# AbbVie-ComputationalGenomics/SAIGEgds

Measured on AMD Instinct MI355X. Metric: variants/sec seqAssocGLMM_SPA at N=430K; achieved HBM GB/s vs roofline, higher is better.
Workload: dtype f64

## Files before the change

### saigegds_amd/csrc/host_lanes.h

```cpp
extern "C" int sgx_set_option(sgx_handle *h, const char *name, long long value)
{
	if (!h || !name) return fail(SGX_EINVAL, "sgx_set_option: NULL argument");
	const std::string n(name);
	if (n == "score_v1") h->force_v1 = value != 0;
	else if (n == "force_dense") h->force_dense = value != 0;
	else if (n == "spa_exact") h->force_exact = value != 0;
	else if (n == "pipe_mb") { if (value < 0 || value > 65536) return fail(SGX_EINVAL, "pipe_mb out of range"); h->pipe_bytes = (size_t)value << 20; return SGX_OK; }
	else if (n == "spa_scan_rows") h->spa_scan_rows = value != 0;
	else if (n == "guard_exp") { if (value < 0 || value > 300) return fail(SGX_EINVAL, "guard_exp must be 0..300"); h->guard_tol = std::pow(10.0, -(double)value); }
	else if (n == "three_plane") { if (value < -1 || value > 1) return fail(SGX_EINVAL, "three_plane must be -1 (automatic), 0 or 1"); h->dense_opt = (int)value; return SGX_OK; }
	else if (n == "lanes") {
		if (value < 1 || value > 4) return fail(SGX_EINVAL, "lanes must be 1..4");
		if (h->owner) return fail(SGX_EINVAL, "lanes: not on a twin");
		int rc = sgx_sync(h);
		if (rc) return rc;
		for (int i = (int)value - 1; i < 3; i++) if (h->twins[i]) { sgx_free(h->twins[i]); h->twins[i] = nullptr; }
		for (int i = 0; i < (int)value - 1; i++) {
			if (h->twins[i]) continue;
			std::unique_ptr<sgx_handle, void (*)(sgx_handle *)> t(new sgx_handle(), sgx_free);
			t->device = h->device; t->md = h->md; t->mf_ok = h->mf_ok; t->mfe = h->mfe; t->dQ = h->dQ;
			for (int g = 0; g < MF_MAXG; g++) { t->mf[g] = h->mf[g]; t->mf_nbfv[g] = h->mf_nbfv[g]; }
			t->owner = h;
			t->force_dense = h->force_dense; t->force_v1 = h->force_v1; t->force_exact = h->force_exact;
			t->spa_scan_rows = h->spa_scan_rows; t->guard_tol = h->guard_tol;
			rc = set_dev(t.get());
			if (!rc) rc = alloc_workspace(t.get());
			if (rc) return rc;
			h->twins[i] = t.release();
		}
		h->n_lanes = (int)value; h->next_lane = 0; h->last_issued = nullptr;
		return SGX_OK;
	}
	else return fail(SGX_EINVAL, "sgx_set_option: unknown option '%s'", name);
	for (sgx_handle *t : h->twins) if (t) { int rc = sgx_set_option(t, name, value); if (rc) return rc; }
	return SGX_OK;
}

static void stats_add(sgx_stats &into, const sgx_stats &x)
{
	into.n_variants += x.n_variants; into.n_valid += x.n_valid; into.n_spa += x.n_spa;
	into.n_spa_dense += x.n_spa_dense; into.n_spa_slow += x.n_spa_slow;
	into.ms_score += x.ms_score; into.ms_spa += x.ms_spa; into.ms_total += x.ms_total;
	into.ms_kernel += x.ms_kernel; into.ms_lists += x.ms_lists;
	into.score_launches += x.score_launches; into.spa_launches += x.spa_launches;
	into.three_plane += x.three_plane; into.n_unlisted += x.n_unlisted; into.n_guarded += x.n_guarded;
}

static int sync_lane(sgx_handle *h)
{
	int rc = set_dev(h);
	if (rc) return rc;
	HIPCHK(hipStreamSynchronize(h->stream));
	if (h->pend_dense.active) {
		h->pend_dense.active = false;
		if (h->stats_pending && h->h_counters[2] > 0) {
			rc = launch_pending_dense(h);
			if (rc) return rc;
			HIPCHK(hipStreamSynchronize(h->stream));
		}
	}
	if (h->stats_pending) {
		h->stats.n_spa = (uint64_t)(h->h_counters[0] + h->h_counters[7] - h->h_counters[6] + h->h_counters[5]);
		h->stats.n_valid = (uint64_t)h->h_counters[1];
		h->stats.n_spa_dense = (uint64_t)h->h_counters[2];
		h->stats.n_spa_slow = (uint64_t)h->h_counters[4];
		h->stats.three_plane = h->form == FORM_THREE ? 1u : 0u;
		h->stats.n_guarded = (uint32_t)h->h_counters[21];
		h->stats.n_unlisted = (uint32_t)h->h_counters[23] - h->stats.n_guarded;
		if (h->form != FORM_FP64) {
			sgx_handle *p = h->owner ? h->owner : h;
			const double frac = 64.0 * (double)h->h_counters[22] / ((double)std::max<uint64_t>(1, h->stats.n_variants) * (double)h->md.N);
			const bool over = (uint64_t)h->stats.n_unlisted * 32 > h->stats.n_variants;
			if (h->form != FORM_THREE && (frac > SGX_DENSE_ON || over)) p->dense_mode = true;
			else if (h->form == FORM_THREE && frac < SGX_DENSE_OFF) p->dense_mode = false;
		}
		float a = 0, b = 0, c = 0;
		(void)hipEventElapsedTime(&a, h->ev[0], h->ev[1]);
		(void)hipEventElapsedTime(&b, h->ev[1], h->ev[2]);
		(void)hipEventElapsedTime(&c, h->ev[0], h->ev[2]);
		h->stats.ms_score = a; h->stats.ms_spa = b; h->stats.ms_total = c;
		float k = 0;
		if (h->evk_set) (void)hipEventElapsedTime(&k, h->evk[0], h->evk[1]);
		h->stats.ms_kernel = k; h->evk_set = false;
		float l = 0;
		if (h->lists_timed) { (void)hipEventElapsedTime(&l, h->ev_lists, h->ev[0]); h->stats.ms_total += l; }
		h->stats.ms_lists = l; h->lists_timed = false;
		h->stats_pending = false;
		sgx_handle *p = h->owner ? h->owner : h;
		stats_add(p->total, h->stats);
		p->total_calls++;
	}
	return SGX_OK;
}

static int begin_call(sgx_handle *h)
{
	const int rc = sync_lane(h);
	if (rc) return rc;
	h->last_issued = h;
	return SGX_OK;
}

extern "C" int sgx_sync(sgx_handle *h)
{
	if (!h) return fail(SGX_EINVAL, "sgx_sync: NULL handle");
	int rc = sync_lane(h);
	for (sgx_handle *t : h->twins) if (!rc && t) rc = sync_lane(t);
	return rc;
}

extern "C" int sgx_get_stats(sgx_handle *h, sgx_stats *st)
{
	if (!h || !st) return fail(SGX_EINVAL, "sgx_get_stats: NULL argument");
	int rc = sgx_sync(h);
	if (rc) return rc;
	*st = (h->last_issued && h->last_issued != h) ? h->last_issued->stats : h->stats;
	return SGX_OK;
}

extern "C" int sgx_get_stats_total(sgx_handle *h, sgx_stats *st, uint64_t *n_calls, int reset)
{
	if (!h || !st) return fail(SGX_EINVAL, "sgx_get_stats_total: NULL argument");
	int rc = sgx_sync(h);
	if (rc) return rc;
	*st = h->total;
	if (n_calls) *n_calls = h->total_calls;
	if (reset) { h->total = sgx_stats{}; h->total_calls = 0; }
	return SGX_OK;
}
```

### saigegds_amd/csrc/host_spa.h

```cpp


template <int LO, typename F, int... I>
static bool with_int(int v, F &&f, std::integer_sequence<int, I...>)
{
	return ((v == LO + I && (f(std::integral_constant<int, LO + I>()), true)) || ...);
}
template <typename F>
static bool with_k(int K, F &&f) { return with_int<1>(K, f, std::make_integer_sequence<int, KMAX>()); }
template <typename F>
static void with_pp(int P, F &&f)
{
	if (P <= 8) f(std::integral_constant<int, 8>());
	else if (P <= 16) f(std::integral_constant<int, 16>());
	else if (P <= 32) f(std::integral_constant<int, 32>());
	else f(std::integral_constant<int, 64>());
}

static dim3 mf_grid(int n_cu, size_t rows, int ntile, int *tps, int vpb = MF_VPB, int wg_per_cu = 2)
{
	const int vt = (int)((rows + vpb - 1) / vpb);
	int sk = std::max(1, (n_cu * wg_per_cu * 4 + vt / 2) / vt);
	sk = std::min(sk, std::max(1, ntile / 24));
	if (sk >= 6) sk = (sk + 7) & ~7;
	sk = std::min(sk, std::max(1, ntile / 2));
	*tps = (ntile + sk - 1) / sk;
	*tps += *tps & 1;
	sk = (ntile + *tps - 1) / *tps;
	return dim3((unsigned)vt, (unsigned)sk);
}

template <int KK, int NCX, int INPUT>
static const void *spa4_moments_fn()
{
	if constexpr (INPUT == IN_2BIT) return (const void *)spa4_moments<KK, NCX>;
	else return (const void *)spa4_moments_ds<KK, NCX, INPUT>;
}

template <int KK, int INPUT>
static void launch_dense(sgx_handle *h, RowsRef rr, size_t M, int slot, const int *list, double *out8)
{
	const dim3 sgrid((unsigned)std::min<size_t>(M, (size_t)h->spa_grid));
	hipLaunchKernelGGL((spa_kernel<KK, 512, INPUT>), sgrid, dim3(512), 0, h->stream, rr,
		h->md, h->recs, h->counters, slot, list, h->scratch, h->scratch_stride, out8);
}

template <int KK, int INPUT>
static int launch_spa_k(sgx_handle *h, RowsRef rr, size_t M, double *out8, bool lazy_dense)
{
	const DevModel &md = h->md;
	hipStream_t st = h->stream;
	if (h->force_v1 && INPUT != IN_2BIT) {
		launch_dense<KK, INPUT>(h, rr, M, 0, nullptr, out8);
		return SGX_OK;
	}
	const size_t fl = spa4_lds_bytes(KK);
	if (!h->mom_attr_set[INPUT]) {
		HIPCHK(hipFuncSetAttribute(spa4_moments_fn<KK, SPA4_NCA, INPUT>(), hipFuncAttributeMaxDynamicSharedMemorySize, (int)fl));
		HIPCHK(hipFuncSetAttribute(spa4_moments_fn<KK, SPA4_NCB, INPUT>(), hipFuncAttributeMaxDynamicSharedMemorySize, (int)fl));
		h->mom_attr_set[INPUT] = true;
	}
	const int nround = (int)((M + h->vcap4 - 1) / h->vcap4);
	const int btop = (int)(2 * M);
	const dim3 gsolve((unsigned)std::min((h->vcap4 + 3) / 4, 4 * h->n_cu));
	const size_t rowb5 = (size_t)((md.N + 63) / 64) * 16;
	const size_t l5 = (INPUT == IN_2BIT && rowb5 <= 120 * 1024) ? rowb5 : 0;
	const bool small5 = INPUT == IN_2BIT && rowb5 <= 32 * 1024;
	if (l5 > 48 * 1024 && !h->spa5_attr_set[INPUT]) {
		HIPCHK(hipFuncSetAttribute((const void *)spa5_kernel<KK, INPUT, 0, 512>, hipFuncAttributeMaxDynamicSharedMemorySize, (int)l5));
		HIPCHK(hipFuncSetAttribute((const void *)spa5_kernel<KK, INPUT, 1, 512>, hipFuncAttributeMaxDynamicSharedMemorySize, (int)l5));
		h->spa5_attr_set[INPUT] = true;
	}
	auto moments = [&](auto ncx, int tier, int rd) {
		constexpr int NCX = decltype(ncx)::value;
		if constexpr (INPUT == IN_2BIT)
			hipLaunchKernelGGL((spa4_moments<KK, NCX>), dim3((unsigned)h->n_cu), dim3(WAVE * spa4_waves(KK)), fl, st, rr, md, h->nseg,
				tier, btop, rd * h->vcap4, h->vcap4, h->recs, h->counters, h->seg4, h->cur5 + 2);
		else
			hipLaunchKernelGGL((spa4_moments_ds<KK, NCX, INPUT>), dim3((unsigned)h->n_cu), dim3(WAVE * spa4_waves(KK)), fl, st,
				(const void *)rr.base, rr.bpv, md, h->nseg, tier, btop, rd * h->vcap4, h->vcap4, h->recs, h->counters, h->seg4, h->cur5 + 2);
		hipLaunchKernelGGL((spa4_solve<KK, NCX>), gsolve, dim3(256), 0, st, md, h->nseg, tier, btop, rd * h->vcap4, h->vcap4,
			h->recs, h->counters, h->seg4, h->fallback, h->fb_x2, out8, h->force_dense ? 1 : 0, h->force_exact ? 1 : 0);
	};
	for (int rd = 0; rd < nround; rd++) moments(std::integral_constant<int, SPA4_NCA>(), 0, rd);
	for (int rd = 0; rd < nround; rd++) moments(std::integral_constant<int, SPA4_NCB>(), 1, rd);
	const size_t ws5 = spa5_wg_bytes(md.N);
	auto spa5 = [&](auto threads, int nwg) {
		constexpr int T5 = decltype(threads)::value;
		if constexpr (T5 == 512 || INPUT == IN_2BIT) {
			hipLaunchKernelGGL((spa5_kernel<KK, INPUT, 0, T5>), dim3((unsigned)nwg), dim3(T5), l5, st, rr, md, h->recs, h->counters,
				h->fb_spa2, h->fb_x2, h->cur5, h->fallback, h->scr5, out8, h->force_dense ? 1 : 0, h->force_exact ? 1 : 0, l5,
				h->spa_scan_rows, ws5, 3);
			hipLaunchKernelGGL((spa5_kernel<KK, INPUT, 1, T5>), dim3((unsigned)nwg), dim3(T5), l5, st, rr, md, h->recs, h->counters,
				h->fb_x2, h->fb_x2, h->cur5 + 1, h->fallback, h->scr5, out8, h->force_dense ? 1 : 0, h->force_exact ? 1 : 0, l5,
				h->spa_scan_rows, ws5, 4);
		}
	};
	if (small5) spa5(std::integral_constant<int, 128>(), h->nwg5);
	else spa5(std::integral_constant<int, 512>(), h->n_cu);
	if (!lazy_dense) launch_dense<KK, INPUT>(h, rr, M, 2, h->fallback, out8);
	return SGX_OK;
}

template <int INPUT>
static int launch_spa(sgx_handle *h, RowsRef rr, size_t M, double *out8, bool lazy_dense = false)
{
	h->stats.spa_launches = 0;
	if (h->md.quant) return SGX_OK;
	int rc = SGX_OK;
	with_k(h->md.K, [&](auto kk) { rc = launch_spa_k<decltype(kk)::value, INPUT>(h, rr, M, out8, lazy_dense); });
	if (rc) return rc;
	HIPCHK(hipGetLastError());
	const bool v1 = h->force_v1 && INPUT != IN_2BIT;
	h->stats.spa_launches = v1 ? 1u : (uint32_t)(4 * ((M + h->vcap4 - 1) / h->vcap4) + 3);
	if (lazy_dense && !v1) { h->pend_dense.active = true; h->pend_dense.rr = rr; h->pend_dense.M = M; h->pend_dense.out8 = out8; }
	return SGX_OK;
}

static int launch_pending_dense(sgx_handle *h)
{
	with_k(h->md.K, [&](auto kk) {
		launch_dense<decltype(kk)::value, IN_2BIT>(h, h->pend_dense.rr, h->pend_dense.M, 2, h->fallback, h->pend_dense.out8);
	});
	HIPCHK(hipGetLastError());
	return SGX_OK;
}

static int scan_begin(sgx_handle *h, hipStream_t sst, ScanForm form, const sgx_block *b)
{
	h->form = form;
	if (b) HIPCHK(hipStreamWaitEvent(sst, b->ready, 0));
	if (form == FORM_FP64) {
		HIPCHK(hipMemsetAsync(h->counters, 0, 24 * sizeof(int), sst));
		if (h->cur5) HIPCHK(hipMemsetAsync(h->cur5, 0, 8 * sizeof(int), sst));
	}
	HIPCHK(hipEventRecord(h->ev[0], sst));
	return SGX_OK;
}

template <int INPUT>
static int scan_end(sgx_handle *h, hipStream_t sst, const sgx_block *b, RowsRef rr, size_t M, double *out8, bool lazy_dense)
{
	HIPCHK(hipEventRecord(h->ev[1], sst));
	h->stats.score_launches = h->form == FORM_FP64 ? 1 : 5;
	if (sst != h->stream) HIPCHK(hipStreamWaitEvent(h->stream, h->ev[1], 0));
	int rc = launch_spa<INPUT>(h, rr, M, out8, lazy_dense);
	if (rc) return rc;
	if (lazy_dense) h->pend_dense.blk = b;
	HIPCHK(hipEventRecord(h->ev[2], h->stream));
	if (b) {
		HIPCHK(hipEventRecord(b->last_read, h->stream));
		const_cast<sgx_block *>(b)->was_read = true;
	}
	HIPCHK(hipMemcpyAsync(h->h_counters, h->counters, 24 * sizeof(int), hipMemcpyDeviceToHost, h->stream));
	h->stats.n_variants = M;
	h->stats_pending = true;
	return SGX_OK;
}

template <int KK, int INPUT>
static int launch_score_fp64(sgx_handle *h, RowsRef rr, size_t M, double *out8, uint8_t *valid)
{
	const DevModel &md = h->md;
	constexpr int SB = 256, P = 2 * KK + 2;
	hipStream_t st = h->stream;
	const dim3 grid((unsigned)M);
	if constexpr (INPUT == IN_2BIT) {
		hipLaunchKernelGGL((score2b_kernel<P, SB>), grid, dim3(SB), 0, st,
			rr, (int)M, md, h->recs, h->counters, out8, valid, (const int *)nullptr, 0, 0, (int *)nullptr, (int *)nullptr);
	} else {
		using T = std::conditional_t<INPUT == IN_U8, uint8_t, double>;
		const T *rows = reinterpret_cast<const T *>(rr.base);
		if constexpr (KK <= 8) {
			if (!h->force_v1) {
				const int vb = (int)((M + DS_TILE_VB - 1) / DS_TILE_VB);
				int ns = std::max(1, std::min((4 * h->n_cu + vb - 1) / vb, (md.N + 4095) / 4096));
				int per = (((md.N + ns - 1) / ns) + 63) & ~63;
				ns = (md.N + per - 1) / per;
				const size_t need = (size_t)ns * M * (3 * P + 2);
				if (need > h->ds_part.cap) {
					HIPCHK(hipStreamSynchronize(st));
					HIPCHK(h->ds_part.reserve(need));
				}
				hipLaunchKernelGGL((score_ds_tile_kernel<P, T>), dim3((unsigned)vb, (unsigned)ns), dim3(256), 0, st,
					rows, (int)M, md, per, h->ds_part);
				hipLaunchKernelGGL((score_ds_tile_epilogue<P>), dim3((unsigned)((M + 255) / 256)), dim3(256), 0, st,
					(int)M, md, ns, h->ds_part, h->recs, h->counters, out8, valid);
				return SGX_OK;
			}
		}
		hipLaunchKernelGGL((score_ds_kernel<P, SB, T>), grid, dim3(SB), 0, st, rows, (int)M, md, h->recs, h->counters, out8, valid);
	}
	return SGX_OK;
}

template <int INPUT>
static int launch_scan(sgx_handle *h, const void *rows, size_t row_bytes, size_t M, double *out8, uint8_t *valid,
	const sgx_block *b = nullptr)
{
	const RowsRef rr{reinterpret_cast<const uint8_t *>(rows), row_bytes, 0, nullptr, nullptr, nullptr};
	int rc = scan_begin(h, h->stream, FORM_FP64, b);
	if (rc) return rc;
	if (!with_k(h->md.K, [&](auto kk) { rc = launch_score_fp64<decltype(kk)::value, INPUT>(h, rr, M, out8, valid); }))
		return fail(SGX_EINVAL, "unsupported K=%d", h->md.K);
	if (rc) return rc;
	HIPCHK(hipGetLastError());
	return scan_end<INPUT>(h, h->stream, b, rr, M, out8, false);
}
```

### saigegds_amd/csrc/kern_spa4.h

```cpp
#pragma once
#include "kern_spa4_tab.h"


__host__ __device__ constexpr int spa4_waves(int) { return 8; }
#define SPA4_NCA 12
#define SPA4_NCB SPA4_NC
#define SPA4_NSMAX (SPA4_NC + 5)
#define SPA4_TAIL_TOL 1e-10

__device__ __forceinline__ double spa4_fma_svv(double a_sgpr, double x, double c_vgpr)
{
	double r;
	asm("v_fma_f64 %0, %1, %2, %3" : "=v"(r) : "s"(a_sgpr), "v"(x), "v"(c_vgpr));
	return r;
}

__device__ __forceinline__ void spa4_max_abs(double &g, double a)
{
	asm("v_max_f64 %0, %0, |%1|" : "+v"(g) : "v"(a));
}

template <int NC>
__device__ __forceinline__ void spa4_cum_terms(double y, double u, double d, double *acc)
{
// ... 260 lines not shown
				};
				fetch_q(ca, lane);
				for (int k0 = 0; k0 < nq; k0 += 2 * WAVE) {
					fetch_q(cb, k0 + WAVE + lane);
					if (ca.ok) work(ca);
					fetch_q(ca, k0 + 2 * WAVE + lane);
					if (cb.ok) work(cb);
				}
				__builtin_amdgcn_wave_barrier();
				fetch(ca);
				while (__ballot(ca.ok)) {
					fetch(cb);
					if (ca.ok) work(ca);
					ca = cb;
				}
			}
			const int idx = wave_reduce_scatter(acc, lane);
			gmax = wave_max_nonneg_to_last(gmax);
			const size_t base = ((size_t)(vb + vl) * nseg + seg) * NS;
			if (!(lane & (NS - 1 > 16 ? 1 : 3)) && idx < NS - 1) segpart[base + idx] = acc[0];
			if (lane == WAVE - 1) segpart[base + (NS - 1)] = gmax;
		}
	}
	spa4_queue_done(cursor);
}

template <int K, int NC, int INPUT>
__global__ void __launch_bounds__(WAVE * spa4_waves(K))
spa4_moments_ds(const void *__restrict__ rows, size_t row_bytes, DevModel md, int nseg, int tier, int btop, int v0, int vcap,
	const SpaRec *__restrict__ recs, const int *__restrict__ counters, double *__restrict__ segpart, int *__restrict__ cursor)
{
	constexpr int SEG = spa_seg(K), KP = (K + 2) & ~1, NS = NC + 5;
	extern __shared__ __attribute__((aligned(16))) uint8_t fill_smem[];
	double *tab = reinterpret_cast<double *>(fill_smem);
	double *pd = tab + (size_t)SEG * KP;
	int *pj = reinterpret_cast<int *>(pd + (size_t)(K + 6) * SPA4_VPER);
	const int N = md.N, tid = threadIdx.x, lane = tid & (WAVE - 1), wid = tid / WAVE;
	const int nflag = min(counters[tier ? 7 : 0] - v0, vcap);
	if (nflag <= 0) return;
	const int vper = spa4_slice(nflag, nseg, gridDim.x, spa4_waves(K));
	const int nslice = (nflag + vper - 1) / vper;
	const int nitem = nseg * nslice;
	__shared__ int sh_it;
	int seg = -1;
	for (;;) {
		__syncthreads();
		if (tid == 0) sh_it = atomicAdd(cursor, 1);
		__syncthreads();
		const int it = sh_it;
		if (it >= nitem) break;
		const int sg = it / nslice, vb = (it - sg * nslice) * vper;
		const int nv = min(vper, nflag - vb);
		if (sg != seg) {
			seg = sg;
			const int nrow = min(SEG, N - seg * SEG);
			spa4_stage_table<spa4_waves(K)>(tab, md.XM + (size_t)seg * SEG * KP, nrow * KP);
		}
		for (int i = tid; i < nv; i += WAVE * spa4_waves(K)) {
			const SpaRec &r = recs[spa4_rec(tier, btop, v0 + vb + i)];
			pj[i] = r.j;
			pj[SPA4_VPER + i] = r.minus;
			pd[i] = 1 / sqrt(r.AC2);
			pd[SPA4_VPER + i] = r.tscale;
#pragma unroll
			for (int a = 0; a < K; a++) pd[(2 + a) * SPA4_VPER + i] = r.c[a];
#pragma unroll
			for (int a = 0; a < 4; a++) pd[(2 + K + a) * SPA4_VPER + i] = r.lut[a];
		}
		__syncthreads();
		const int s_lo = seg * SEG, nstep = (min(SEG, N - s_lo) + WAVE - 1) / WAVE;
		for (int vl = wid; vl < nv; vl += spa4_waves(K)) {
			const double inv = pd[vl], ts = pd[SPA4_VPER + vl];
			const double imp = pd[(2 + K + 3) * SPA4_VPER + vl];
			const bool minus = pj[SPA4_VPER + vl] != 0;
			const uint8_t *row = reinterpret_cast<const uint8_t *>(rows) + (size_t)pj[vl] * row_bytes;
			double c[K];
#pragma unroll
			for (int a = 0; a < K; a++) c[a] = pd[(2 + a) * SPA4_VPER + vl];
			double acc[NS - 1], gmax = 0;
#pragma unroll
			for (int a = 0; a < NS - 1; a++) acc[a] = 0;
			auto dosage = [&](int j) -> double {
				const int i = s_lo + j * WAVE + lane;
				if (i >= N) return 0.0;
				if (INPUT == IN_U8) {
					const uint8_t v = row[i];
					return (v == 0xFF) ? imp : (minus ? 2.0 - (double)v : (double)v);
				} else {
					const double v = reinterpret_cast<const double *>(row)[i];
					return !isfinite(v) ? imp : (minus ? 2.0 - v : v);
				}
			};
			double gn = dosage(0);
			for (int j = 0; j < nstep; j++) {
				const double G = gn;
				if (j + 1 < nstep) gn = dosage(j + 1);
				if (G != 0) spa4_carrier<K, NC>(tab + (size_t)(j * WAVE + lane) * KP, G, c, inv, ts, acc, gmax);
			}
			const int idx = wave_reduce_scatter(acc, lane);
			gmax = wave_max_nonneg_to_last(gmax);
			const size_t base = ((size_t)(vb + vl) * nseg + seg) * NS;
			if (!(lane & (NS - 1 > 16 ? 1 : 3)) && idx < NS - 1) segpart[base + idx] = acc[0];
			if (lane == WAVE - 1) segpart[base + (NS - 1)] = gmax;
		}
	}
	spa4_queue_done(cursor);
}

template <int NC>
struct Spa4Series {
	double k1, k2;
	double kp[NC - 2];
	double ts, gmax;
};

template <int NC>
__device__ __forceinline__ bool spa4_eval(const Spa4Series<NC> &S, double xmax, double t, double &K1s, double &K2s, double &K0s)
{
	const double its = 1 / S.ts, tau = t * its;
	double p0 = 0, p1 = 0, p2 = 0;
#pragma unroll
	for (int n = NC; n >= 3; n--) {
		const double kn = S.kp[n - 3];
		p0 = fma(p0, tau, kn);
		p1 = fma(p1, tau, (double)n * kn);
		p2 = fma(p2, tau, (double)(n * (n - 1)) * kn);
	}
	const double tau2 = tau * tau;
	K0s = fma(t, S.k1, fma(0.5 * t * t, S.k2, p0 * tau2 * tau));
	K1s = S.k1 + fma(t, S.k2, p1 * tau2 * its);
	K2s = fma(p2 * tau, its * its, S.k2);
	double tp = tau;
#pragma unroll
	for (int k = 1; k < NC - 3; k++) tp *= tau;
	const double tail = (fabs((double)(NC * (NC - 1)) * S.kp[NC - 3] * tp * tau) +
		fabs((double)((NC - 1) * (NC - 2)) * S.kp[NC - 4] * tp)) * its * its;
	return S.gmax * fabs(t) <= xmax && tail <= SPA4_TAIL_TOL * fabs(K2s) && isfinite(K2s);
}

template <int NC>
__device__ __forceinline__ bool spa4_root(const Spa4Series<NC> &S, double xmax, double q, double NAmu, double NAsigma, RootState &s)
{
	root_begin(s, q, 0, 0);
	root_feed(s, S.k1, S.k2, NAmu, NAsigma, 0.0, true);
	while (s.active) {
		double K1s, K2s, K0s;
		if (!spa4_eval(S, xmax, s.tnew, K1s, K2s, K0s)) return false;
		root_feed(s, K1s, K2s, NAmu, NAsigma, K0s, true);
	}
	return true;
}

template <int K, int NC>
__device__ __forceinline__ void spa4_solve_one(const DevModel &md, int nseg, int tier, int btop, int v0, int vcap, int v, int lane,
	SpaRec *__restrict__ recs, int *__restrict__ counters, const double *__restrict__ segpart,
	int *__restrict__ fb_dense, int *__restrict__ fb_exact, double *__restrict__ out8, int force_dense, int force_exact);

template <int K, int NC>
__global__ void __launch_bounds__(256)
spa4_solve(DevModel md, int nseg, int tier, int btop, int v0, int vcap, SpaRec *__restrict__ recs, int *__restrict__ counters,
	const double *__restrict__ segpart, int *__restrict__ fb_dense, int *__restrict__ fb_exact,
	double *__restrict__ out8, int force_dense, int force_exact)
{
	const int lane = threadIdx.x & (WAVE - 1);
	const int nflag = min(counters[tier ? 7 : 0] - v0, vcap);
	for (int v = (blockIdx.x * blockDim.x + threadIdx.x) / WAVE; v < nflag; v += gridDim.x * blockDim.x / WAVE)
		spa4_solve_one<K, NC>(md, nseg, tier, btop, v0, vcap, v, lane, recs, counters, segpart, fb_dense, fb_exact, out8,
			force_dense, force_exact);
}

template <int K, int NC>
__device__ __forceinline__ void spa4_solve_one(const DevModel &md, int nseg, int tier, int btop, int v0, int vcap, int v, int lane,
	SpaRec *__restrict__ recs, int *__restrict__ counters, const double *__restrict__ segpart,
	int *__restrict__ fb_dense, int *__restrict__ fb_exact, double *__restrict__ out8, int force_dense, int force_exact)
{
	constexpr int NS = NC + 5;
	const int ri = spa4_rec(tier, btop, v0 + v);
	const SpaRec r = recs[ri];
	double a[NS];
#pragma unroll
	for (int x = 0; x < NS; x++) a[x] = 0;
	for (int s = lane; s < nseg; s += WAVE) {
		const double *p = segpart + ((size_t)v * nseg + s) * NS;
#pragma unroll
		for (int x = 0; x < NS - 1; x++) a[x] += p[x];
		a[NS - 1] = fmax(a[NS - 1], p[NS - 1]);
	}
#pragma unroll
	for (int x = 0; x < NS - 1; x++) a[x] = wave_sum(a[x]);
#pragma unroll
	for (int o = 32; o > 0; o >>= 1) a[NS - 1] = fmax(a[NS - 1], __shfl_xor(a[NS - 1], o, WAVE));
	if (lane > 1) return;
	const double inv = 1 / sqrt(r.AC2);
	double xmu_c = 0, xsum_c = 0;
#pragma unroll
	for (int x = 0; x < K; x++) { xmu_c = fma(md.Xmu[x], r.c[x], xmu_c); xsum_c = fma(md.Xsum[x], r.c[x], xsum_c); }
	const double Tstat = r.S * inv;
	const double var2 = r.var2 / r.AC2, var1 = var2 * md.r;
	const double m1 = (a[0] - xmu_c) * inv;
	const double qtilde = Tstat / sqrt(var1) * sqrt(var2) + m1;
	const double sdev = qtilde - m1, qinv = -sdev + m1;
	const double pn_in = d_pchisq1_upper(sdev * sdev / var2);
	if (fabs(qtilde - m1) / sqrt(var2) < 2.0) {
		if (lane == 0) spa_write_row(r, Tstat, var1, pn_in, true, out8);
		return;
	}
	const double nb = (xsum_c - a[1]) * inv;
	const double L = a[2] + fmax(-nb, 0.0), U = a[3] + fmin(-nb, 0.0);
	const double mar = 1e-9 * (fabs(L) + fabs(U) + fabs(qtilde) + fabs(qinv));
	if (force_dense || !(qtilde < L - mar && qtilde > U + mar && qinv < L - mar && qinv > U + mar)) {
		if (lane == 0) fb_dense[atomicAdd(&counters[2], 1)] = ri;
		return;
	}
	Spa4Series<NC> S;
	S.k1 = a[4]; S.k2 = a[5]; S.ts = r.tscale; S.gmax = a[NS - 1];
#pragma unroll
	for (int x = 0; x < NC - 2; x++) S.kp[x] = a[6 + x];
	const double NAmu = m1 - a[4], NAsigma = var2 - a[5];
	const double qmine = lane == 0 ? qtilde : qinv;
	RootState sm;
	const bool ok_mine = !force_exact && spa4_root(S, md.spa_xmax, qmine, NAmu, NAsigma, sm);
	double p_mine = 0;
	if (ok_mine && sm.converged) p_mine = lugannani_rice(sm.root, sm.Kcur, sm.K2cur, qmine, NAmu, NAsigma);
	const int st_mine = (ok_mine ? 1 : 0) | (ok_mine && sm.converged ? 2 : 0);
	const double p_other = __shfl(p_mine, 1, WAVE);
	const int st_other = __shfl(st_mine, 1, WAVE);
	if (lane != 0) return;
	if (!(st_mine & 1) || !(st_other & 1)) {
		if (tier == 0 && !force_exact) {
			const int slot = atomicAdd(&counters[7], 1);
			atomicAdd(&counters[6], 1);
			recs[btop - 1 - slot] = r;
		} else {
			fb_exact[atomicAdd(&counters[4], 1)] = ri;
		}
		return;
	}
	bool converged;
	const double pval = spa_two_roots(p_mine, p_other, (st_mine & 2) && (st_other & 2), pn_in, converged);
	spa_write_row(r, Tstat, var1, pval, converged, out8);
}


#define SPA5_BIG 2048

__device__ __forceinline__ void cgf_terms_rt(double g, double m, double t, bool with_k, double &k1, double &k2, double &k0)
{
	const double om = 1 - m, mg = m * g, c2 = om * mg * g;
	const double e = fast_exp(-g * t);
	const double d = fma(om, e, m);
	const double rr = isfinite(d) ? fast_rcp(d) : 0.0;
	k1 = fma(mg, rr, k1);
	const double tt = c2 * e * rr * rr;
	if (isfinite(tt)) k2 += tt;
	if (with_k) k0 += cgf_korg_term(g, m, t, d, om);
}

__host__ __device__ inline size_t spa5_wg_bytes(int N) { return (((size_t)N + 63) & ~(size_t)63) * (16 + 4); }

template <int BLOCK>
__device__ __noinline__ void spa5_cum_sweep(const double2 *__restrict__ glist, int nnz, double ts, double *kp_out)
{
	constexpr int NC = SPA4_NCB;
	double kp[NC - 1];
#pragma unroll
	for (int a = 0; a < NC - 1; a++) kp[a] = 0;
	double2 gn = (int)threadIdx.x < nnz ? glist[threadIdx.x] : make_double2(0.0, 0.5);
	for (int k = threadIdx.x; k < nnz; k += BLOCK) {
		const double2 gm = gn;
		if (k + BLOCK < nnz) gn = glist[k + BLOCK];
		const double mui = gm.y;
		spa4_cum_terms<NC>(gm.x * ts, mui * (1 - mui), 1 - 2 * mui, kp);
		kp[NC - 2] = fmax(kp[NC - 2], fabs(gm.x));
	}
#pragma unroll
	for (int a = 0; a < NC - 1; a++) kp_out[a] = kp[a];
}

__device__ __noinline__ int spa5_series_solve(const double *arg, const SpaRec *__restrict__ rec, double *__restrict__ out8)
{
	constexpr int NC = SPA4_NCB;
	Spa4Series<NC> S;
#pragma unroll
	for (int a = 0; a < NC - 2; a++) S.kp[a] = arg[a];
	S.k1 = arg[NC - 2]; S.k2 = arg[NC - 1]; S.ts = arg[NC]; S.gmax = arg[NC + 1];
	const double xmax = arg[NC + 2], qtilde = arg[NC + 3], qinv = arg[NC + 4], NAmu = arg[NC + 5], NAsigma = arg[NC + 6];
	const double pn_in = arg[NC + 7], Tstat = arg[NC + 8], var1 = arg[NC + 9];
	RootState s1, s2;
	if (!spa4_root(S, xmax, qtilde, NAmu, NAsigma, s1) || !spa4_root(S, xmax, qinv, NAmu, NAsigma, s2)) return 0;
	const bool both = s1.converged && s2.converged;
	double p1 = 0, p2 = 0;
	if (both) {
		p1 = lugannani_rice(s1.root, s1.Kcur, s1.K2cur, qtilde, NAmu, NAsigma);
		p2 = lugannani_rice(s2.root, s2.Kcur, s2.K2cur, qinv, NAmu, NAsigma);
	}
	bool converged;
	const double pval = spa_two_roots(p1, p2, both, pn_in, converged);
	const SpaRec rr = *rec;
	spa_write_row(rr, Tstat, var1, pval, converged, out8);
	return 1;
}

template <int BLOCK>
__device__ __forceinline__ bool spa5_series(const double2 *__restrict__ glist, int nnz, double ts, double xmax,
	double k1, double k2, double qtilde, double qinv, double NAmu, double NAsigma, double pn_in,
	double Tstat, double var1, const SpaRec *__restrict__ rec, double *__restrict__ out8, double *sh, int *sh_flag)
{
	constexpr int NC = SPA4_NCB;
	double kp[NC - 1];
	spa5_cum_sweep<BLOCK>(glist, nnz, ts, kp);
	constexpr int NWV = BLOCK / WAVE;
	double gmax = kp[NC - 2];
	const int lane = threadIdx.x & (WAVE - 1), wv = threadIdx.x / WAVE;
	double kr[NC - 2];
#pragma unroll
	for (int a = 0; a < NC - 2; a++) kr[a] = kp[a];
	const int idx = wave_reduce_scatter(kr, lane);
#pragma unroll
	for (int o = 32; o > 0; o >>= 1) gmax = fmax(gmax, __shfl_xor(gmax, o, WAVE));
	double *part = sh + NC + 16;
	if (!(lane & 3) && idx < NC - 2) part[idx * NWV + wv] = kr[0];
	if (lane == 1) part[(NC - 2) * NWV + wv] = gmax;
	__syncthreads();
	double *arg = sh;
	if (threadIdx.x < NC - 2) {
		double t = 0;
		for (int w = 0; w < NWV; w++) t += part[threadIdx.x * NWV + w];
		arg[threadIdx.x] = t;
	}
	__syncthreads();
	if (threadIdx.x == 0) {
		for (int w = 0; w < NWV; w++) gmax = fmax(gmax, part[(NC - 2) * NWV + w]);
		arg[NC - 2] = k1; arg[NC - 1] = k2; arg[NC] = ts; arg[NC + 1] = gmax; arg[NC + 2] = xmax;
		arg[NC + 3] = qtilde; arg[NC + 4] = qinv; arg[NC + 5] = NAmu; arg[NC + 6] = NAsigma;
		arg[NC + 7] = pn_in; arg[NC + 8] = Tstat; arg[NC + 9] = var1;
		*sh_flag = spa5_series_solve(arg, rec, out8);
	}
	__syncthreads();
	const bool done = *sh_flag != 0;
	__syncthreads();
	return done;
}

__host__ __device__ constexpr int spa5_waves_per_simd(int BLOCK) { return BLOCK == 512 ? 2 : (BLOCK / 64 + 3) / 4; }
template <int K, int INPUT, int MODE, int BLOCK>
__global__ void __launch_bounds__(BLOCK, spa5_waves_per_simd(BLOCK))
spa5_kernel(RowsRef rr, DevModel md, const SpaRec *__restrict__ recs,
	int *__restrict__ counters, const int *__restrict__ todo, int *__restrict__ todo_next, int *__restrict__ cursor,
	int *__restrict__ fb_dense, uint8_t *__restrict__ scratch, double *__restrict__ out8, int force_dense, int force_exact,
	size_t lds_row_bytes, bool scan_rows, size_t wg_stride, int nslot)
{
	constexpr int KP = (K + 2) & ~1, NW = BLOCK / WAVE;
	extern __shared__ __attribute__((aligned(16))) uint8_t fill_smem[];
	uint4 *rows_lds = reinterpret_cast<uint4 *>(fill_smem);
	__shared__ double sh[SPA4_NCB * NW + SPA4_NCB + 16];
	__shared__ int sh_flag;
	__shared__ int shi[NW];
	__shared__ int sh_vi, sh_v;
	__shared__ SpaRec sh_rec;
	const int N = md.N, tid = threadIdx.x, lane = tid & (WAVE - 1), wid = tid / WAVE;
	double2 *glist = reinterpret_cast<double2 *>(scratch + (size_t)blockIdx.x * wg_stride);
	uint32_t *ilist = reinterpret_cast<uint32_t *>(glist + (((size_t)N + 63) & ~(size_t)63));
	const int ntodo = counters[nslot];
	const int nvec = INPUT == IN_2BIT ? (int)(min((size_t)((N + 63) >> 6) * 16, rr_row_bytes(rr)) / 16) : (N + 63) >> 6;
	const int per = ((nvec + NW - 1) / NW + WAVE - 1) & ~(WAVE - 1);
	for (;;) {
		__syncthreads();
		if (tid < WAVE) {
			int vi0 = 0;
			if (tid == 0) vi0 = atomicAdd(cursor, 1);
			vi0 = __builtin_amdgcn_readfirstlane(vi0);
			int v0 = -1;
			if (vi0 < 2 * ntodo) {
				v0 = todo[vi0 < ntodo ? vi0 : vi0 - ntodo];
				const double *src = reinterpret_cast<const double *>(recs + v0);
				for (int i = tid; i < (int)(sizeof(SpaRec) / 8); i += WAVE) reinterpret_cast<double *>(&sh_rec)[i] = src[i];
			}
			if (tid == 0) { sh_vi = vi0; sh_v = v0; }
		}
		__syncthreads();
		const int vi = sh_vi;
		if (vi >= 2 * ntodo) break;
		const bool big_round = vi < ntodo;
		const int v = sh_v;
		const SpaRec &r = sh_rec;
		if ((r.nnz > SPA5_BIG) != big_round) continue;
		auto row_piece = [&](int p) -> uint4 { return *reinterpret_cast<const uint4 *>(rr.base + rr_piece(rr, (size_t)r.j, (size_t)p)); };
		const uint32_t zx = r.minus ? 0xAAAAAAAAu : 0u;
		const double lut0 = r.lut[0], lut1 = r.lut[1], lut2 = r.lut[2], lut3 = r.lut[3];
		const bool listed = INPUT == IN_2BIT && !scan_rows && rr.cptr != nullptr && rr.corient[r.j] == (r.minus ? 2 : 1);
		const uint32_t *il = listed ? rr.cidx + rr.cptr[r.j] : ilist;
		int nnz = listed ? r.nnz : 0;
		if (!listed) {
			const bool staged = INPUT == IN_2BIT && lds_row_bytes >= (size_t)nvec * 16;
			if (staged) {
				constexpr int UN = 8;
				for (int p0 = tid; p0 < nvec; p0 += UN * BLOCK) {
					uint4 t[UN];
	#pragma unroll
					for (int j = 0; j < UN; j++) { const int p = p0 + j * BLOCK; t[j] = p < nvec ? row_piece(p) : make_uint4(0u, 0u, 0u, 0u); }
	#pragma unroll
					for (int j = 0; j < UN; j++) { const int p = p0 + j * BLOCK; if (p < nvec) rows_lds[p] = t[j]; }
				}
				__syncthreads();
			}
			auto masks = [&](int p, uint32_t (&ww)[4], uint32_t (&z)[4]) -> int {
				int cnt = 0;
				if (INPUT == IN_2BIT) {
					uint4 w = make_uint4(0u, 0u, 0u, 0u);
					if (p < nvec) w = staged ? rows_lds[p] : row_piece(p);
					ww[0] = w.x; ww[1] = w.y; ww[2] = w.z; ww[3] = w.w;
	#pragma unroll
					for (int k = 0; k < 4; k++) { z[k] = nz_fields((ww[k] ^ zx) & keep_mask(N - p * 64 - 16 * k)); cnt += __popc(z[k]); }
				} else {
					z[0] = z[1] = z[2] = z[3] = 0;
					if (p < nvec) {
						for (int s2 = 0; s2 < 64; s2++) {
							const int i = p * 64 + s2;
							if (i < N && load_dosage<INPUT>(rr, i, r) != 0) { z[s2 >> 5] |= 1u << (s2 & 31); cnt++; }
						}
					}
				}
				return cnt;
			};
			int cnt_w = 0;
			for (int it = 0; it < per; it += WAVE) {
				uint32_t ww[4], z[4];
				cnt_w += masks(wid * per + it + lane, ww, z);
			}
			cnt_w = wave_sum_i(cnt_w);
			if (lane == 0) shi[wid] = cnt_w;
			__syncthreads();
			int o_w = 0;
	#pragma unroll
			for (int w = 0; w < NW; w++) { if (w < wid) o_w += shi[w]; nnz += shi[w]; }
			for (int it = 0; it < per; it += WAVE) {
				uint32_t ww[4], z[4];
				const int p = wid * per + it + lane;
				const int cnt = masks(p, ww, z);
				if (!__ballot(cnt != 0)) continue;
				int incl = cnt;
	#pragma unroll
				for (int o = 1; o < WAVE; o <<= 1) {
					const int up = __shfl_up(incl, o, WAVE);
					if (lane >= o) incl += up;
				}
				int o2 = o_w + incl - cnt;
				o_w += __shfl(incl, WAVE - 1, WAVE);
				if (INPUT == IN_2BIT) {
	#pragma unroll
					for (int k = 0; k < 4; k++) {
						uint32_t zz = z[k];
						while (zz) {
							const int b = __ffs(zz) - 1;
							zz &= zz - 1;
							ilist[o2++] = (uint32_t)(p * 64 + 16 * k + (b >> 1)) | (((ww[k] >> b) & 3u) << 30);
						}
					}
				} else {
	#pragma unroll
					for (int k = 0; k < 2; k++) {
						uint32_t zz = z[k];
						while (zz) {
							const int b = __ffs(zz) - 1;
							zz &= zz - 1;
							ilist[o2++] = (uint32_t)(p * 64 + 32 * k + b);
						}
					}
				}
			}
			__syncthreads();
		}
		const double inv = 1 / sqrt(r.AC2);
		double c[K];
#pragma unroll
		for (int a = 0; a < K; a++) c[a] = r.c[a];
		double a6[6] = {0, 0, 0, 0, 0, 0};
		constexpr int UNG = K <= 4 ? 4 : 2;
		for (int k0 = tid; k0 < nnz; k0 += UNG * BLOCK) {
			uint32_t e[UNG];
			double xv[UNG][KP];
#pragma unroll
			for (int j = 0; j < UNG; j++) e[j] = (k0 + j * BLOCK < nnz) ? il[k0 + j * BLOCK] : 0u;
#pragma unroll
			for (int j = 0; j < UNG; j++) {
				const double *x = md.XM + (size_t)(e[j] & 0x3FFFFFFFu) * KP;
#pragma unroll
				for (int a = 0; a < KP; a += 2) {
					const double2 t2 = *reinterpret_cast<const double2 *>(x + a);
					xv[j][a] = t2.x; xv[j][a + 1] = t2.y;
				}
			}
#pragma unroll
			for (int j = 0; j < UNG; j++) {
				const int k = k0 + j * BLOCK;
				if (k >= nnz) continue;
				const uint32_t code = e[j] >> 30;
				const double G = INPUT == IN_2BIT ? ((code & 2u) ? ((code & 1u) ? lut3 : lut2) : ((code & 1u) ? lut1 : lut0))
					: load_dosage<INPUT>(rr, (int)(e[j] & 0x3FFFFFFFu), r);
				double b = 0;
#pragma unroll
				for (int a = 0; a < K; a++) b = fma(xv[j][a], c[a], b);
				const double mui = xv[j][K];
				const double adj = (G - b) * inv;
				glist[k] = make_double2(adj, mui);
				a6[0] = fma(mui, G, a6[0]);
				a6[1] += b;
				if (adj > 0) a6[2] += adj; else a6[3] += adj;
				a6[4] = fma(adj, mui, a6[4]);
				a6[5] = fma(adj * adj, mui * (1 - mui), a6[5]);
			}
		}
		block_sum<6, BLOCK>(a6, sh);
		double xmu_c = 0, xsum_c = 0;
#pragma unroll
		for (int a = 0; a < K; a++) { xmu_c = fma(md.Xmu[a], c[a], xmu_c); xsum_c = fma(md.Xsum[a], c[a], xsum_c); }
		const double m1 = (a6[0] - xmu_c) * inv;
		const double Tstat = r.S * inv;
		const double var2 = r.var2 / r.AC2, var1 = var2 * md.r;
		const double qtilde = Tstat / sqrt(var1) * sqrt(var2) + m1;
		const double sdev = qtilde - m1, qinv = -sdev + m1;
		const double pn_in = d_pchisq1_upper(sdev * sdev / var2);
		double pval;
		bool converged = true;
		if (fabs(qtilde - m1) / sqrt(var2) < 2.0) {
			pval = pn_in;
		} else {
			const double nb = (xsum_c - a6[1]) * inv;
			const double L = a6[2] + fmax(-nb, 0.0), U = a6[3] + fmin(-nb, 0.0);
			const double mar = 1e-9 * (fabs(L) + fabs(U) + fabs(qtilde) + fabs(qinv));
			if (force_dense || !(qtilde < L - mar && qtilde > U + mar && qinv < L - mar && qinv > U + mar)) {
				if (tid == 0) fb_dense[atomicAdd(&counters[2], 1)] = v;
				continue;
			}
			const double NAmu = m1 - a6[4], NAsigma = var2 - a6[5];
			if (MODE == 0) {
				if (force_exact || !spa5_series<BLOCK>(glist, nnz, r.tscale, md.spa_xmax, a6[4], a6[5], qtilde, qinv, NAmu, NAsigma,
						pn_in, Tstat, var1, &sh_rec, out8, sh, &sh_flag)) {
					if (tid == 0) todo_next[atomicAdd(&counters[4], 1)] = v;
				}
				continue;
			}
			RootState s1, s2;
			root_begin(s1, qtilde, L, U);
			root_begin(s2, qinv, L, U);
			root_feed(s1, a6[4], a6[5], NAmu, NAsigma, 0.0, true);
			root_feed(s2, a6[4], a6[5], NAmu, NAsigma, 0.0, true);
			auto sweep = [&](bool a1, bool a2, bool k1w, bool k2w, double t1, double t2, double (&sv)[6]) {
#pragma unroll
				for (int a = 0; a < 6; a++) sv[a] = 0;
				double2 gn = tid < nnz ? glist[tid] : make_double2(0.0, 0.5);
				for (int k0 = tid; k0 < nnz; k0 += BLOCK) {
					const double2 gm = gn;
					if (k0 + BLOCK < nnz) gn = glist[k0 + BLOCK];
					if (a1) cgf_terms_rt(gm.x, gm.y, t1, k1w, sv[0], sv[1], sv[2]);
					if (a2) cgf_terms_rt(gm.x, gm.y, t2, k2w, sv[3], sv[4], sv[5]);
				}
				block_sum<6, BLOCK>(sv, sh);
			};
			while (s1.active || s2.active) {
				const bool a1 = s1.active, a2 = s2.active, k1w = s1.want_k, k2w = s2.want_k;
				double sv[6];
				sweep(a1, a2, k1w, k2w, s1.tnew, s2.tnew, sv);
				if (a1) root_feed(s1, sv[0], sv[1], NAmu, NAsigma, sv[2], k1w);
				if (a2) root_feed(s2, sv[3], sv[4], NAmu, NAsigma, sv[5], k2w);
			}
			const bool both = s1.converged && s2.converged;
			double p1 = 0, p2 = 0;
			if (both) {
				if (!(s1.k_ok && s2.k_ok)) {
					double sv[6];
					sweep(!s1.k_ok, !s2.k_ok, true, true, s1.root, s2.root, sv);
					if (!s1.k_ok) s1.Kcur = sv[2];
					if (!s2.k_ok) s2.Kcur = sv[5];
				}
				p1 = lugannani_rice(s1.root, s1.Kcur, s1.K2cur, qtilde, NAmu, NAsigma);
				p2 = lugannani_rice(s2.root, s2.Kcur, s2.K2cur, qinv, NAmu, NAsigma);
			}
			pval = spa_two_roots(p1, p2, both, pn_in, converged);
		}
		if (tid == 0) spa_write_row(r, Tstat, var1, pval, converged, out8);
	}
}
```

Baseline: 18.34 million.

## Merge two-pass spa5 kernels into one launch with inline exact fallback

Replaces the two spa5 launches (series mode, then exact mode on leftovers) with a single kernel. It walks the combined todo list from both queues, tries the series approximation, and on failure runs the exact root-finding in place instead of deferring the variant to a second launch. The series and exact paths become noinline device functions, which is meant to cut register pressure in the main loop and save one launch plus the re-staging of genotype rows. The cost is possible load imbalance, since slow exact work now mixes with fast series work inside one launch, plus call overhead at the noinline boundaries.

```diff
diff --git a/saigegds_amd/csrc/host_lanes.h b/saigegds_amd/csrc/host_lanes.h
--- a/saigegds_amd/csrc/host_lanes.h
+++ b/saigegds_amd/csrc/host_lanes.h
@@ -63,7 +63,7 @@
 		h->stats.n_spa = (uint64_t)(h->h_counters[0] + h->h_counters[7] - h->h_counters[6] + h->h_counters[5]);
 		h->stats.n_valid = (uint64_t)h->h_counters[1];
 		h->stats.n_spa_dense = (uint64_t)h->h_counters[2];
-		h->stats.n_spa_slow = (uint64_t)h->h_counters[4];
+		h->stats.n_spa_slow = (uint64_t)(h->h_counters[4] + h->h_counters[8]);
 		h->stats.three_plane = h->form == FORM_THREE ? 1u : 0u;
 		h->stats.n_guarded = (uint32_t)h->h_counters[21];
 		h->stats.n_unlisted = (uint32_t)h->h_counters[23] - h->stats.n_guarded;
diff --git a/saigegds_amd/csrc/host_spa.h b/saigegds_amd/csrc/host_spa.h
--- a/saigegds_amd/csrc/host_spa.h
+++ b/saigegds_amd/csrc/host_spa.h
@@ -66,18 +66,17 @@
 	const size_t l5 = (INPUT == IN_2BIT && rowb5 <= 120 * 1024) ? rowb5 : 0;
 	const bool small5 = INPUT == IN_2BIT && rowb5 <= 32 * 1024;
 	if (l5 > 48 * 1024 && !h->spa5_attr_set[INPUT]) {
-		HIPCHK(hipFuncSetAttribute((const void *)spa5_kernel<KK, INPUT, 0, 512>, hipFuncAttributeMaxDynamicSharedMemorySize, (int)l5));
-		HIPCHK(hipFuncSetAttribute((const void *)spa5_kernel<KK, INPUT, 1, 512>, hipFuncAttributeMaxDynamicSharedMemorySize, (int)l5));
+		HIPCHK(hipFuncSetAttribute((const void *)spa5_kernel<KK, INPUT, 512>, hipFuncAttributeMaxDynamicSharedMemorySize, (int)l5));
 		h->spa5_attr_set[INPUT] = true;
 	}
 	auto moments = [&](auto ncx, int tier, int rd) {
 		constexpr int NCX = decltype(ncx)::value;
 		if constexpr (INPUT == IN_2BIT)
 			hipLaunchKernelGGL((spa4_moments<KK, NCX>), dim3((unsigned)h->n_cu), dim3(WAVE * spa4_waves(KK)), fl, st, rr, md, h->nseg,
-				tier, btop, rd * h->vcap4, h->vcap4, h->recs, h->counters, h->seg4, h->cur5 + 2);
+				tier, btop, rd * h->vcap4, h->vcap4, h->recs, h->counters, h->seg4, h->cur5 + 1);
 		else
 			hipLaunchKernelGGL((spa4_moments_ds<KK, NCX, INPUT>), dim3((unsigned)h->n_cu), dim3(WAVE * spa4_waves(KK)), fl, st,
-				(const void *)rr.base, rr.bpv, md, h->nseg, tier, btop, rd * h->vcap4, h->vcap4, h->recs, h->counters, h->seg4, h->cur5 + 2);
+				(const void *)rr.base, rr.bpv, md, h->nseg, tier, btop, rd * h->vcap4, h->vcap4, h->recs, h->counters, h->seg4, h->cur5 + 1);
 		hipLaunchKernelGGL((spa4_solve<KK, NCX>), gsolve, dim3(256), 0, st, md, h->nseg, tier, btop, rd * h->vcap4, h->vcap4,
 			h->recs, h->counters, h->seg4, h->fallback, h->fb_x2, out8, h->force_dense ? 1 : 0, h->force_exact ? 1 : 0);
 	};
@@ -86,14 +85,10 @@
 	const size_t ws5 = spa5_wg_bytes(md.N);
 	auto spa5 = [&](auto threads, int nwg) {
 		constexpr int T5 = decltype(threads)::value;
-		if constexpr (T5 == 512 || INPUT == IN_2BIT) {
-			hipLaunchKernelGGL((spa5_kernel<KK, INPUT, 0, T5>), dim3((unsigned)nwg), dim3(T5), l5, st, rr, md, h->recs, h->counters,
-				h->fb_spa2, h->fb_x2, h->cur5, h->fallback, h->scr5, out8, h->force_dense ? 1 : 0, h->force_exact ? 1 : 0, l5,
-				h->spa_scan_rows, ws5, 3);
-			hipLaunchKernelGGL((spa5_kernel<KK, INPUT, 1, T5>), dim3((unsigned)nwg), dim3(T5), l5, st, rr, md, h->recs, h->counters,
-				h->fb_x2, h->fb_x2, h->cur5 + 1, h->fallback, h->scr5, out8, h->force_dense ? 1 : 0, h->force_exact ? 1 : 0, l5,
-				h->spa_scan_rows, ws5, 4);
-		}
+		if constexpr (T5 == 512 || INPUT == IN_2BIT)
+			hipLaunchKernelGGL((spa5_kernel<KK, INPUT, T5>), dim3((unsigned)nwg), dim3(T5), l5, st, rr, md, h->recs, h->counters,
+				h->fb_x2, h->fb_spa2, h->cur5, h->fallback, h->scr5, out8, h->force_dense ? 1 : 0, h->force_exact ? 1 : 0, l5,
+				h->spa_scan_rows, ws5);
 	};
 	if (small5) spa5(std::integral_constant<int, 128>(), h->nwg5);
 	else spa5(std::integral_constant<int, 512>(), h->n_cu);
@@ -111,7 +106,7 @@
 	if (rc) return rc;
 	HIPCHK(hipGetLastError());
 	const bool v1 = h->force_v1 && INPUT != IN_2BIT;
-	h->stats.spa_launches = v1 ? 1u : (uint32_t)(4 * ((M + h->vcap4 - 1) / h->vcap4) + 3);
+	h->stats.spa_launches = v1 ? 1u : (uint32_t)(4 * ((M + h->vcap4 - 1) / h->vcap4) + 2);
 	if (lazy_dense && !v1) { h->pend_dense.active = true; h->pend_dense.rr = rr; h->pend_dense.M = M; h->pend_dense.out8 = out8; }
 	return SGX_OK;
 }
diff --git a/saigegds_amd/csrc/kern_spa4.h b/saigegds_amd/csrc/kern_spa4.h
--- a/saigegds_amd/csrc/kern_spa4.h
+++ b/saigegds_amd/csrc/kern_spa4.h
@@ -586,7 +586,7 @@
 }
 
 template <int BLOCK>
-__device__ __forceinline__ bool spa5_series(const double2 *__restrict__ glist, int nnz, double ts, double xmax,
+__device__ __noinline__ bool spa5_series(const double2 *__restrict__ glist, int nnz, double ts, double xmax,
 	double k1, double k2, double qtilde, double qinv, double NAmu, double NAsigma, double pn_in,
 	double Tstat, double var1, const SpaRec *__restrict__ rec, double *__restrict__ out8, double *sh, int *sh_flag)
 {
@@ -626,13 +626,56 @@
 	return done;
 }
 
+template <int BLOCK>
+__device__ __noinline__ double spa5_exact(const double2 *__restrict__ glist, int nnz, double k1, double k2, double qtilde, double qinv,
+	double L, double U, double NAmu, double NAsigma, double pn_in, double *sh, bool &converged)
+{
+	RootState s1, s2;
+	root_begin(s1, qtilde, L, U);
+	root_begin(s2, qinv, L, U);
+	root_feed(s1, k1, k2, NAmu, NAsigma, 0.0, true);
+	root_feed(s2, k1, k2, NAmu, NAsigma, 0.0, true);
+	auto sweep = [&](bool a1, bool a2, bool k1w, bool k2w, double t1, double t2, double (&sv)[6]) {
+#pragma unroll
+		for (int a = 0; a < 6; a++) sv[a] = 0;
+		double2 gn = (int)threadIdx.x < nnz ? glist[(int)threadIdx.x] : make_double2(0.0, 0.5);
+		for (int k0 = (int)threadIdx.x; k0 < nnz; k0 += BLOCK) {
+			const double2 gm = gn;
+			if (k0 + BLOCK < nnz) gn = glist[k0 + BLOCK];
+			if (a1) cgf_terms_rt(gm.x, gm.y, t1, k1w, sv[0], sv[1], sv[2]);
+			if (a2) cgf_terms_rt(gm.x, gm.y, t2, k2w, sv[3], sv[4], sv[5]);
+		}
+		block_sum<6, BLOCK>(sv, sh);
+	};
+	while (s1.active || s2.active) {
+		const bool a1 = s1.active, a2 = s2.active, k1w = s1.want_k, k2w = s2.want_k;
+		double sv[6];
+		sweep(a1, a2, k1w, k2w, s1.tnew, s2.tnew, sv);
+		if (a1) root_feed(s1, sv[0], sv[1], NAmu, NAsigma, sv[2], k1w);
+		if (a2) root_feed(s2, sv[3], sv[4], NAmu, NAsigma, sv[5], k2w);
+	}
+	const bool both = s1.converged && s2.converged;
+	double p1 = 0, p2 = 0;
+	if (both) {
+		if (!(s1.k_ok && s2.k_ok)) {
+			double sv[6];
+			sweep(!s1.k_ok, !s2.k_ok, true, true, s1.root, s2.root, sv);
+			if (!s1.k_ok) s1.Kcur = sv[2];
+			if (!s2.k_ok) s2.Kcur = sv[5];
+		}
+		p1 = lugannani_rice(s1.root, s1.Kcur, s1.K2cur, qtilde, NAmu, NAsigma);
+		p2 = lugannani_rice(s2.root, s2.Kcur, s2.K2cur, qinv, NAmu, NAsigma);
+	}
+	return spa_two_roots(p1, p2, both, pn_in, converged);
+}
+
 __host__ __device__ constexpr int spa5_waves_per_simd(int BLOCK) { return BLOCK == 512 ? 2 : (BLOCK / 64 + 3) / 4; }
-template <int K, int INPUT, int MODE, int BLOCK>
+template <int K, int INPUT, int BLOCK>
 __global__ void __launch_bounds__(BLOCK, spa5_waves_per_simd(BLOCK))
 spa5_kernel(RowsRef rr, DevModel md, const SpaRec *__restrict__ recs,
-	int *__restrict__ counters, const int *__restrict__ todo, int *__restrict__ todo_next, int *__restrict__ cursor,
+	int *__restrict__ counters, const int *__restrict__ todo_x, const int *__restrict__ todo_s, int *__restrict__ cursor,
 	int *__restrict__ fb_dense, uint8_t *__restrict__ scratch, double *__restrict__ out8, int force_dense, int force_exact,
-	size_t lds_row_bytes, bool scan_rows, size_t wg_stride, int nslot)
+	size_t lds_row_bytes, bool scan_rows, size_t wg_stride)
 {
 	constexpr int KP = (K + 2) & ~1, NW = BLOCK / WAVE;
 	extern __shared__ __attribute__((aligned(16))) uint8_t fill_smem[];
@@ -645,7 +688,7 @@
 	const int N = md.N, tid = threadIdx.x, lane = tid & (WAVE - 1), wid = tid / WAVE;
 	double2 *glist = reinterpret_cast<double2 *>(scratch + (size_t)blockIdx.x * wg_stride);
 	uint32_t *ilist = reinterpret_cast<uint32_t *>(glist + (((size_t)N + 63) & ~(size_t)63));
-	const int ntodo = counters[nslot];
+	const int nx = counters[4], ntodo = nx + counters[3];
 	const int nvec = INPUT == IN_2BIT ? (int)(min((size_t)((N + 63) >> 6) * 16, rr_row_bytes(rr)) / 16) : (N + 63) >> 6;
 	const int per = ((nvec + NW - 1) / NW + WAVE - 1) & ~(WAVE - 1);
 	for (;;) {
@@ -656,7 +699,8 @@
 			vi0 = __builtin_amdgcn_readfirstlane(vi0);
 			int v0 = -1;
 			if (vi0 < 2 * ntodo) {
-				v0 = todo[vi0 < ntodo ? vi0 : vi0 - ntodo];
+				const int q = vi0 < ntodo ? vi0 : vi0 - ntodo;
+				v0 = q < nx ? todo_x[q] : todo_s[q - nx];
 				const double *src = reinterpret_cast<const double *>(recs + v0);
 				for (int i = tid; i < (int)(sizeof(SpaRec) / 8); i += WAVE) reinterpret_cast<double *>(&sh_rec)[i] = src[i];
 			}
@@ -818,50 +862,13 @@
 				continue;
 			}
 			const double NAmu = m1 - a6[4], NAsigma = var2 - a6[5];
-			if (MODE == 0) {
-				if (force_exact || !spa5_series<BLOCK>(glist, nnz, r.tscale, md.spa_xmax, a6[4], a6[5], qtilde, qinv, NAmu, NAsigma,
-						pn_in, Tstat, var1, &sh_rec, out8, sh, &sh_flag)) {
-					if (tid == 0) todo_next[atomicAdd(&counters[4], 1)] = v;
-				}
-				continue;
-			}
-			RootState s1, s2;
-			root_begin(s1, qtilde, L, U);
-			root_begin(s2, qinv, L, U);
-			root_feed(s1, a6[4], a6[5], NAmu, NAsigma, 0.0, true);
-			root_feed(s2, a6[4], a6[5], NAmu, NAsigma, 0.0, true);
-			auto sweep = [&](bool a1, bool a2, bool k1w, bool k2w, double t1, double t2, double (&sv)[6]) {
-#pragma unroll
-				for (int a = 0; a < 6; a++) sv[a] = 0;
-				double2 gn = tid < nnz ? glist[tid] : make_double2(0.0, 0.5);
-				for (int k0 = tid; k0 < nnz; k0 += BLOCK) {
-					const double2 gm = gn;
-					if (k0 + BLOCK < nnz) gn = glist[k0 + BLOCK];
-					if (a1) cgf_terms_rt(gm.x, gm.y, t1, k1w, sv[0], sv[1], sv[2]);
-					if (a2) cgf_terms_rt(gm.x, gm.y, t2, k2w, sv[3], sv[4], sv[5]);
-				}
-				block_sum<6, BLOCK>(sv, sh);
-			};
-			while (s1.active || s2.active) {
-				const bool a1 = s1.active, a2 = s2.active, k1w = s1.want_k, k2w = s2.want_k;
-				double sv[6];
-				sweep(a1, a2, k1w, k2w, s1.tnew, s2.tnew, sv);
-				if (a1) root_feed(s1, sv[0], sv[1], NAmu, NAsigma, sv[2], k1w);
-				if (a2) root_feed(s2, sv[3], sv[4], NAmu, NAsigma, sv[5], k2w);
-			}
-			const bool both = s1.converged && s2.converged;
-			double p1 = 0, p2 = 0;
-			if (both) {
-				if (!(s1.k_ok && s2.k_ok)) {
-					double sv[6];
-					sweep(!s1.k_ok, !s2.k_ok, true, true, s1.root, s2.root, sv);
-					if (!s1.k_ok) s1.Kcur = sv[2];
-					if (!s2.k_ok) s2.Kcur = sv[5];
-				}
-				p1 = lugannani_rice(s1.root, s1.Kcur, s1.K2cur, qtilde, NAmu, NAsigma);
-				p2 = lugannani_rice(s2.root, s2.Kcur, s2.K2cur, qinv, NAmu, NAsigma);
-			}
-			pval = spa_two_roots(p1, p2, both, pn_in, converged);
+			if ((big_round ? vi : vi - ntodo) >= nx) {
+				if (!force_exact && spa5_series<BLOCK>(glist, nnz, r.tscale, md.spa_xmax, a6[4], a6[5], qtilde, qinv, NAmu, NAsigma,
+						pn_in, Tstat, var1, &sh_rec, out8, sh, &sh_flag))
+					continue;
+				if (tid == 0) atomicAdd(&counters[8], 1);
+			}
+			pval = spa5_exact<BLOCK>(glist, nnz, a6[4], a6[5], qtilde, qinv, L, U, NAmu, NAsigma, pn_in, sh, converged);
 		}
 		if (tid == 0) spa_write_row(r, Tstat, var1, pval, converged, out8);
 	}
```

Result: slower. 17.42 million (-5.0%).
